# yeyupiaoling/PPASR

Hardware: NVIDIA B200
Metric: utterances_per_sec (higher is better)
Workload: dtype bf16

## Files before the change

### include/ppasr_b200.h

```cpp
#ifndef PPASR_B200_H_
#define PPASR_B200_H_

#include <stdint.h>

#ifdef __cplusplus
extern "C" {
#endif

typedef struct ppasr_b200_ctx ppasr_b200_ctx;

typedef struct ppasr_b200_config {
  int32_t model_type;
  int32_t feat_dim;
  int32_t d_model;
  int32_t n_heads;
  int32_t ffn_dim;
  int32_t n_layers;
  int32_t conv_kernel;
  int32_t causal;
  int32_t conv_norm;
  int32_t vocab_size;
  int32_t max_len;
  int32_t reduce_idx;
  int32_t recover_idx;
// ... 53 lines not shown
int64_t ppasr_b200_beam_workspace_bytes(int32_t B, int32_t T);
int ppasr_b200_beam_reset(void* states, int32_t B, int32_t max_frames, int32_t beam, void* stream);
int ppasr_b200_beam_advance(const float* probs, int32_t B, int32_t T, int32_t V, const int32_t* frame_lens,
                            int32_t beam, float cutoff_prob, int32_t cutoff_top_n, int32_t blank_id, void* states,
                            int32_t max_frames, void* workspace, void* stream);
int ppasr_b200_beam_advance_lm(const float* probs, int32_t B, int32_t T, int32_t V, const int32_t* frame_lens, int32_t beam,
                               float cutoff_prob, int32_t cutoff_top_n, int32_t blank_id, void* states, int32_t max_frames,
                               void* workspace, const uint64_t* lm_keys, const uint32_t* lm_keys_hi, const float* lm_vals,
                               const int32_t* lm_in_vocab, int64_t lm_capacity, int32_t lm_order, float alpha, float beta,
                               void* stream);
int ppasr_b200_beam_result(const void* states, int32_t B, int32_t max_frames, int32_t beam, int32_t* out_ids,
                           int32_t lmax, int32_t* out_lens, float* out_scores, void* stream);
int ppasr_b200_beam_result_nbest(const void* states, int32_t B, int32_t max_frames, int32_t beam, int32_t nbest,
                                 int32_t* out_ids, int32_t lmax, int32_t* out_lens, float* out_scores, void* stream);
int ppasr_b200_op_ctc_prune(const float* probs, int32_t rows, int32_t V, float cutoff_prob, int32_t cutoff_top_n,
                            void* workspace, void* stream);

int ppasr_b200_op_linear(const void* a_bf16, int64_t lda, const void* w_bf16, int64_t w_rows, const float* bias,
                         void* out, int64_t ldo, int32_t M, int32_t N, int32_t K, int32_t epilogue, int32_t act,
                         float alpha, int32_t residual, const int32_t* lens, int32_t T, int32_t block_n, void* stream);
int ppasr_b200_op_layernorm(float* x, void* y_bf16, const float* g1, const float* b1, const float* g2,
                            const float* b2, const int32_t* lens, int32_t T, int32_t M, int32_t D, float eps,
                            void* stream);
int ppasr_b200_op_dwconv(const void* g_bf16, const float* w, const float* bias, const float* pad_left,
                         const float* gamma, const float* beta, int32_t use_layer_norm, void* out_bf16, int32_t B,
                         int32_t Tin, int32_t Tout, int32_t C, int32_t K, int32_t lpad, float eps, void* stream);
int ppasr_b200_op_softmax(const float* logits, int32_t ldl, float* probs, int32_t M, int32_t V, void* stream);
int ppasr_b200_op_fused_ffn(const void* y_bf16, const void* w1_bf16, const void* w2s_bf16, float* x, void* y_out,
                            const float* b1, const float* b2s, const float* g1, const float* bn1, const float* g2,
                            const float* bn2, int32_t M, int32_t FF, float eps, void* stream);
int ppasr_b200_op_attention(const void* q2, const void* kk, const void* vt, int32_t T2p, const void* pos,
                            int32_t pos_rows, int32_t pos_ld, int32_t pos_row0, int32_t pos_col0, void* out,
                            int32_t B, int32_t H, int32_t T1, int32_t T2, const int32_t* klens, void* stream);
int ppasr_b200_op_grouped_attention(const void* q2g, const void* kk, int32_t k_pitch, const void* vt, int32_t vt_pitch,
                                    const void* pos, void* out, int32_t B, int32_t H, int32_t T, int32_t Tgk,
                                    const int32_t* klens, void* stream);

int ppasr_b200_fbank_frames(int32_t n_samples);
int ppasr_b200_fbank(const float* audio, int32_t B, int64_t stride, int32_t N, const int32_t* n_samples, int32_t n_mels,
                     int32_t sample_rate, int32_t db_normalize, float target_db, float* gain_ws, float* out, int32_t Tmax,
                     void* stream);

int ppasr_b200_set_option(ppasr_b200_ctx* ctx, const char* name, int32_t value);

int ppasr_b200_graph_begin(ppasr_b200_ctx* ctx, void* stream);
int ppasr_b200_graph_end(ppasr_b200_ctx* ctx, void* stream);
int ppasr_b200_graph_launch(ppasr_b200_ctx* ctx, void* stream);
int32_t ppasr_b200_graph_kernels(const ppasr_b200_ctx* ctx);

int ppasr_b200_profile_enable(ppasr_b200_ctx* ctx, int32_t enable);
int ppasr_b200_profile_num_classes(void);
const char* ppasr_b200_profile_class_name(int32_t cls);
int ppasr_b200_profile_read(ppasr_b200_ctx* ctx, int32_t* counts, float* total_ms);

int ppasr_b200_debug_copy_x(ppasr_b200_ctx* ctx, float* dst_device, void* stream);
int ppasr_b200_debug_copy_phase(ppasr_b200_ctx* ctx, void* dst_device, int32_t* dims, void* stream);

#ifdef __cplusplus
}
#endif
#endif
```

### ppasr_b200/_lib.py

```python
import ctypes
import os

_HERE = os.path.dirname(os.path.abspath(__file__))
LIB_PATH = os.path.join(_HERE, "lib", "libppasr_b200.so")

c_void_p = ctypes.c_void_p
c_int = ctypes.c_int
c_int64 = ctypes.c_int64
c_float = ctypes.c_float
c_char_p = ctypes.c_char_p

_lib = None


class PPASRB200Error(Exception):
    """Raised when a C-ABI call returns a non-zero status (message from ppasr_b200_last_error)."""


def load():
    global _lib
    if _lib is not None:
        return _lib
    if not os.path.exists(LIB_PATH):
        raise PPASRB200Error(
# ... 26 lines not shown
    "ppasr_b200_destroy": (c_int, [P]),
    "ppasr_b200_load_tensor": (c_int, [P, c_char_p, P, I, P]),
    "ppasr_b200_finalize": (c_int, [P]),
    "ppasr_b200_encode": (c_int, [P, P, I, P, I, I, P]),
    "ppasr_b200_out_frames": (c_int, [P, I]),
    "ppasr_b200_ctc_probs": (c_int, [P, P, I, P]),
    "ppasr_b200_ctc_logits": (c_int, [P, P, I, P]),
    "ppasr_b200_ctc_greedy": (c_int, [P, P, P, P, P, P, I, I, I, P]),
    "ppasr_b200_stream_reset": (c_int, [P, I]),
    "ppasr_b200_encode_chunk": (c_int, [P, P, I, I, I, I, P]),
    "ppasr_b200_stream_info": (c_int, [P, P, P]),
    "ppasr_b200_sessions_init": (c_int, [P, I]),
    "ppasr_b200_sessions_reset": (c_int, [P, I]),
    "ppasr_b200_sessions_step": (c_int, [P, P, I, P, I, I, I, P]),
    "ppasr_b200_fbank_frames": (c_int, [I]),
    "ppasr_b200_fbank": (c_int, [P, I, c_int64, I, P, I, I, I, c_float, P, P, I, P]),
    "ppasr_b200_ds2_states": (c_int, [P, P, P, I, P]),
    "ppasr_b200_stream_export": (c_int, [P, P, P, I, P]),
    "ppasr_b200_beam_state_bytes": (c_int64, [I, I, I]),
    "ppasr_b200_beam_workspace_bytes": (c_int64, [I, I]),
    "ppasr_b200_beam_reset": (c_int, [P, I, I, I, P]),
    "ppasr_b200_beam_advance": (c_int, [P, I, I, I, P, I, c_float, I, I, P, I, P, P]),
    "ppasr_b200_beam_advance_lm": (c_int, [P, I, I, I, P, I, c_float, I, I, P, I, P, P, P, P, P, c_int64, I, c_float, c_float, P]),
    "ppasr_b200_beam_result": (c_int, [P, I, I, I, P, I, P, P, P]),
    "ppasr_b200_beam_result_nbest": (c_int, [P, I, I, I, I, P, I, P, P, P]),
    "ppasr_b200_op_ctc_prune": (c_int, [P, I, I, c_float, I, P, P]),
    "ppasr_b200_greedy_decode": (c_int, [P, I, I, I, P, I, P, I, P, P, P, P, P]),
    "ppasr_b200_op_linear": (c_int, [P, c_int64, P, c_int64, P, P, c_int64, I, I, I, I, I, c_float, I, P, I, I, P]),
    "ppasr_b200_op_layernorm": (c_int, [P, P, P, P, P, P, P, I, I, I, c_float, P]),
    "ppasr_b200_op_dwconv": (c_int, [P, P, P, P, P, P, I, P, I, I, I, I, I, I, c_float, P]),
    "ppasr_b200_op_softmax": (c_int, [P, I, P, I, I, P]),
    "ppasr_b200_op_fused_ffn": (c_int, [P, P, P, P, P, P, P, P, P, P, P, I, I, c_float, P]),
    "ppasr_b200_op_attention": (c_int, [P, P, P, I, P, I, I, I, I, P, I, I, I, I, P, P]),
    "ppasr_b200_op_grouped_attention": (c_int, [P, P, I, P, I, P, P, I, I, I, I, P, P]),
    "ppasr_b200_debug_copy_x": (c_int, [P, P, P]),
    "ppasr_b200_debug_copy_phase": (c_int, [P, P, P, P]),
    "ppasr_b200_set_option": (c_int, [P, c_char_p, I]),
    "ppasr_b200_graph_begin": (c_int, [P, P]),
    "ppasr_b200_graph_end": (c_int, [P, P]),
    "ppasr_b200_graph_launch": (c_int, [P, P]),
    "ppasr_b200_graph_kernels": (c_int, [P]),
    "ppasr_b200_profile_enable": (c_int, [P, I]),
    "ppasr_b200_profile_num_classes": (c_int, []),
    "ppasr_b200_profile_class_name": (c_char_p, [I]),
    "ppasr_b200_profile_read": (c_int, [P, P, P]),
}


def _declare(lib):
    for name, (res, args) in PROTOTYPES.items():
        fn = getattr(lib, name)
        fn.restype = res
        fn.argtypes = args


def ptr(t):
    if t is None:
        return None
    return c_void_p(t.data_ptr())


def stream_ptr(stream=None):
    import torch
    s = stream if stream is not None else torch.cuda.current_stream()
    return c_void_p(s.cuda_stream)
```

### ppasr_b200/csrc/attention.cu

```cuda
#include "kernels.h"
#include "launch.h"
#include "ptx.cuh"

namespace ppasr {

void count_launch();

constexpr int ATT_BM = 128;
constexpr int ATT_BN = 128;
constexpr int ATT_THREADS = 288;
constexpr int ATT_TILE_BYTES = 128 * 64 * 2;
constexpr int ATT_SMEM_Q = 0;
constexpr int ATT_SMEM_KP = 2 * ATT_TILE_BYTES;
constexpr int ATT_SMEM_V = 4 * ATT_TILE_BYTES;
constexpr int ATT_SMEM_BAR = 5 * ATT_TILE_BYTES;
constexpr int ATT_SMEM_XCH = ATT_SMEM_BAR + 128;
constexpr int ATT_SMEM_TOTAL = ATT_SMEM_XCH + 1024 + 1024;
constexpr int ATT_TMEM_COLS = 256;

__global__ void __launch_bounds__(ATT_THREADS, 2)
rel_attention_kernel(const __grid_constant__ CUtensorMap tm_q, const __grid_constant__ CUtensorMap tm_k,
                     const __grid_constant__ CUtensorMap tm_p, const __grid_constant__ CUtensorMap tm_vt,
                     const AttnParams p) {
  extern __shared__ uint8_t smem_raw[];
// ... 175 lines not shown
      const float inv = l_run > 0.f ? 1.0f / l_run : 0.f;
      uint32_t pk[16];
#pragma unroll
      for (int i = 0; i < 16; ++i) pk[i] = pack_bf16x2(o[2 * i] * inv, o[2 * i + 1] * inv);
      uint4* dst = reinterpret_cast<uint4*>(p.out + ((size_t)b * p.T1 + t) * p.D + h * 64 + ch * 32);
#pragma unroll
      for (int i = 0; i < 4; ++i) dst[i] = make_uint4(pk[4 * i], pk[4 * i + 1], pk[4 * i + 2], pk[4 * i + 3]);
    }
  }

  tc_fence_before();
  __syncthreads();
  if (warp_idx == 8) {
    tc_fence_after();
    tmem_dealloc<ATT_TMEM_COLS>(tmem_base);
  }
}

cudaError_t launch_rel_attention(const CUtensorMap& tm_q, const CUtensorMap& tm_k, const CUtensorMap& tm_p,
                                 const CUtensorMap& tm_vt, const AttnParams& p, cudaStream_t st) {
  static bool configured = false;
  if (!configured) {
    cudaError_t e = cudaFuncSetAttribute(rel_attention_kernel, cudaFuncAttributeMaxDynamicSharedMemorySize,
                                         ATT_SMEM_TOTAL);
    if (e != cudaSuccess) return e;
    configured = true;
  }
  dim3 grid((p.T1 + ATT_BM - 1) / ATT_BM, p.H, p.B);
  cudaError_t le = launch_pdl(rel_attention_kernel, grid, dim3(ATT_THREADS), (size_t)ATT_SMEM_TOTAL, st, tm_q, tm_k, tm_p, tm_vt, p);
  count_launch();
  return le != cudaSuccess ? le : cudaGetLastError();
}

}
```

### ppasr_b200/csrc/kernels.h

```cpp
#pragma once
#include <cuda.h>
#include <cuda_bf16.h>
#include <cuda_runtime.h>
#include <stdint.h>

namespace ppasr {

cudaError_t launch_layernorm(float* x, __nv_bfloat16* y, const float* g1, const float* b1, const float* g2,
                             const float* b2, const int* lens, int T, int M, int D, float eps, cudaStream_t st);

cudaError_t launch_conv1_subsample(const float* feats, const float* mean, const float* istd, const float* w,
                                   const float* bias, __nv_bfloat16* out, int B, int T, int F, int C, int T1, int F1,
                                   int Th, int FH, cudaStream_t st);

cudaError_t launch_conv1_tc(const CUtensorMap& tmap_phase, const float* feats, const float* mean, const float* istd,
                            const float* w, const float* bias, int B, int T, int F, int T1, int F1, int Th, int FH,
                            int num_sms, cudaStream_t st);

cudaError_t launch_conv_front_tc(const CUtensorMap& tmap_w2, const float* feats, const float* mean, const float* istd,
                                 const float* w1, const float* b1, const float* b2, __nv_bfloat16* out, int B, int T, int F,
                                 int T1, int F1, int Th, int FH, int Tout, int Fout, int num_sms, cudaStream_t st);

cudaError_t launch_dwconv_norm_swish(const __nv_bfloat16* g, const float* w, const float* bias, const float* pad_left,
                                     const float* gamma, const float* beta, int use_layer_norm, __nv_bfloat16* out,
// ... 69 lines not shown
  float alpha, beta;
};
size_t beam_state_stride(int node_cap);
cudaError_t launch_ctc_prune(const float* probs, int V, int rows, float cutoff_prob, int top_n, int* cnt, int* cid,
                             float* clp, cudaStream_t st);
cudaError_t launch_beam_reset(void* states, int B, int node_cap, cudaStream_t st);
cudaError_t launch_beam_advance(const int* cnt, const int* cid, const float* clp, int B, int T, const int* frame_lens,
                                int beam, int topn, int blank, int max_frames, void* states, int node_cap, cudaStream_t st,
                                const float* probs = nullptr, int V = 0, const BeamLm* lm = nullptr);
cudaError_t launch_beam_result(const void* states, int B, int node_cap, int nbest, int* out_ids, int lmax, int* out_lens,
                               float* out_scores, cudaStream_t st);
constexpr int BEAM_MAX_TOPN = 64;
constexpr int BEAM_MAX_BEAM = 512;

struct AttnParams {
  int B, H;
  int T1;
  int T2;
  int q_rows_per_bh;
  int k_rows_per_bh;
  int k_row0;
  int pos_row0;
  int pos_col0;
  int D;
  const int* klens;
  const int* slots;
  const int* k_row0s;
  const int* pos_row0s;
  __nv_bfloat16* out;
};
cudaError_t launch_rel_attention(const CUtensorMap& tm_q, const CUtensorMap& tm_k, const CUtensorMap& tm_p,
                                 const CUtensorMap& tm_vt, const AttnParams& p, cudaStream_t st);


struct GroupedAttnParams {
  int B, H;
  int T;
  int Tg;
  const int* klens;
  __nv_bfloat16* out;
  int Tgk = 0;
  int k_pitch = 0;
};
cudaError_t launch_grouped_attention(const CUtensorMap& tm_q, const CUtensorMap& tm_k, const CUtensorMap& tm_p,
                                     const CUtensorMap& tm_vt, const GroupedAttnParams& p, cudaStream_t st);
cudaError_t launch_grouped_pos(const __nv_bfloat16* tab, int ldtab, int col0, int T, int Tpad, __nv_bfloat16* out,
                               cudaStream_t st);
cudaError_t launch_dwconv_stride(const __nv_bfloat16* g, const float* w, const float* bias, const float* pad_left,
                                 const float* ng, const float* nb, int layer_norm, __nv_bfloat16* z, int B, int T, int Tout,
                                 int C, int K, int lpad, int stride, float eps, const int* zero_lens, cudaStream_t st);
cudaError_t launch_avgpool2(const float* x, float* out, int B, int T, int Tout, int C, cudaStream_t st);

}
```

### ppasr_b200/csrc/runtime.cu

```cuda
#include <cmath>
#include <cstdlib>
#include <cstring>
#include <map>
#include <string>
#include <vector>

#include "common.h"
#include "gemm.cuh"
#include "kernels.h"
#include "ppasr_b200.h"
#include "tmap.h"

namespace ppasr {

GemmShape make_shape(int M, int N, int K, int block_n);

struct HostTensor {
  std::vector<float> data;
  std::vector<int64_t> shape;
  int64_t numel() const {
    int64_t n = 1;
    for (auto s : shape) n *= s;
    return n;
  }
// ... 6 lines not shown
  cudaError_t reserve(size_t bytes) {
    if (bytes <= cap) return cudaSuccess;
    if (base) cudaFree(base);
    base = nullptr;
    cap = 0;
    cudaError_t e = cudaMalloc(&base, bytes);
    if (e == cudaSuccess) cap = bytes;
    return e;
  }
  void rewind() { used = 0, overflow = false; }
  template <class T>
  T* take(size_t count) {
    const size_t off = (used + 255) & ~size_t(255);
    if (overflow || off + count * sizeof(T) > cap) {
      overflow = true;
      return nullptr;
    }
    used = off + count * sizeof(T);
    return reinterpret_cast<T*>(base + off);
  }
  void release() {
    if (base) cudaFree(base);
    base = nullptr;
    cap = used = 0;
  }
};

struct BlockW {
  const __nv_bfloat16 *wqkv, *wo, *pw1, *pw2;
  const float *bqkv, *bo, *pos_u, *pos_v, *pw1_b, *pw2_b, *dw_w, *dw_b, *cn_g, *cn_b, *glu_pad;
};
struct BlockMaps {
  CUtensorMap wqkv, wo, pw1, pw2;
};

struct LayerW : BlockW {
  const float *ln_ffm_g, *ln_ffm_b, *ln_mha_g, *ln_mha_b, *ln_conv_g, *ln_conv_b, *ln_ff_g, *ln_ff_b, *ln_fin_g,
      *ln_fin_b;
  const __nv_bfloat16 *ffm_w1, *ff_w1, *ffm_w2s, *ff_w2s;
  const float *ffm_b1, *ff_b1, *ffm_b2s, *ff_b2s;
};

struct Plan {
  int B = 0, T = 0, T1 = 0, Tp = 0, Th = 0, M = 0, Mr = 0, Tkp = 0;
  float* feats = nullptr;
  int* vlen = nullptr;
  __nv_bfloat16 *phase = nullptr, *c2 = nullptr, *y = nullptr, *q2 = nullptr, *kk = nullptr, *vt = nullptr,
                *att = nullptr, *g = nullptr, *z = nullptr;
  int Mc = 0, Tc = 0;
  int* vc = nullptr;
  int Tg = 0, Tgp = 0;
  __nv_bfloat16 *q2g = nullptr, *kkg = nullptr, *vtg = nullptr, *pg = nullptr;
  CUtensorMap tm_qg, tm_kg, tm_vtg, tm_pg[4];
  float *x2 = nullptr;
  int* vlen2 = nullptr;
  float *x = nullptr, *logits = nullptr, *pmax = nullptr, *psum = nullptr, *maxp = nullptr, *score = nullptr,
        *probs = nullptr;
  int *parg = nullptr, *idx = nullptr, *ids = nullptr, *out_len = nullptr;
  int Tcat = 0, Mcat = 0;
  __nv_bfloat16 *ycat = nullptr, *gcat = nullptr;
  CUtensorMap tm_phase, tm_c2, tm_y, tm_att, tm_g, tm_z, tm_q, tm_k, tm_vt, tm_ycat;
};

}

using namespace ppasr;
// ... 275 lines not shown
  return PPASR_OK;
}

int pack_attention(ppasr_b200_ctx* c, const std::string& p, int l, bool grouped, bool pos_bias, BlockW& w, BlockMaps& m,
                   std::vector<float>& wpos_all, std::vector<float>& bpos_all) {
  const int D = c->cfg.d_model;
  PPASR_REQUIRE(c->host[p + "self_attn.pos_bias_u"].numel() == (int64_t)c->cfg.n_heads * (grouped ? 192 : 64) &&
                    c->host[p + "self_attn.pos_bias_v"].numel() == (int64_t)c->cfg.n_heads * (grouped ? 192 : 64),
                "pos_bias_u / pos_bias_v shape");
  {
    std::vector<float> qkv((size_t)3 * D * D), bq((size_t)3 * D);
    const char* nm[3] = {"linear_q", "linear_k", "linear_v"};
    for (int s = 0; s < 3; ++s) {
      auto t = transpose_in_out(c->host[p + "self_attn." + nm[s] + ".weight"]);
      std::memcpy(qkv.data() + (size_t)s * D * D, t.data(), sizeof(float) * D * D);
      std::memcpy(bq.data() + (size_t)s * D, c->host[p + "self_attn." + nm[s] + ".bias"].data.data(), sizeof(float) * D);
    }
    w.wqkv = upload(c, to_bf16(qkv));
    w.bqkv = upload(c, bq);
  }
  w.wo = upload(c, to_bf16(transpose_in_out(c->host[p + "self_attn.linear_out.weight"])));
  w.bo = vecf(c, p + "self_attn.linear_out.bias");
  w.pos_u = vecf(c, p + "self_attn.pos_bias_u");
  w.pos_v = vecf(c, p + "self_attn.pos_bias_v");
  {
    auto t = transpose_in_out(c->host[p + "self_attn.linear_pos.weight"]);
    std::memcpy(wpos_all.data() + (size_t)l * D * D, t.data(), sizeof(float) * D * D);
    if (pos_bias)
      std::memcpy(bpos_all.data() + (size_t)l * D, c->host[p + "self_attn.linear_pos.bias"].data.data(), sizeof(float) * D);
  }
  if (int rc = check_weights(c)) return rc;
  std::string err;
  if (!make_tmap_2d(&m.wqkv, w.wqkv, D, 3 * D, (uint64_t)D * 2, BN_NARROW, &err) ||
      !make_tmap_2d(&m.wo, w.wo, D, D, (uint64_t)D * 2, BN_WIDE, &err)) {
    set_last_error(err);
    return PPASR_ERR_CUDA;
  }
  return PPASR_OK;
}

int pack_conv_module(ppasr_b200_ctx* c, const std::string& p, int K, BlockW& w, BlockMaps& m) {
  const auto& cfg = c->cfg;
  const int D = cfg.d_model;
  {
    const HostTensor& pw = c->host[p + "conv_module.pointwise_conv1.weight"];
    const HostTensor& pb = c->host[p + "conv_module.pointwise_conv1.bias"];
    PPASR_REQUIRE(pw.numel() == (int64_t)2 * D * D, "pointwise_conv1.weight shape");
    std::vector<float> wi((size_t)2 * D * D), bi((size_t)2 * D);
    for (int ch = 0; ch < D; ++ch) {
      std::memcpy(&wi[(size_t)(2 * ch) * D], &pw.data[(size_t)ch * D], sizeof(float) * D);
      std::memcpy(&wi[(size_t)(2 * ch + 1) * D], &pw.data[(size_t)(ch + D) * D], sizeof(float) * D);
      bi[2 * ch] = pb.data[ch];
      bi[2 * ch + 1] = pb.data[ch + D];
    }
    w.pw1 = upload(c, to_bf16(wi));
    w.pw1_b = upload(c, bi);
  }
  float* pad = c->wslab.take<float>(D);
  {
    const HostTensor& dw = c->host[p + "conv_module.depthwise_conv.weight"];
    PPASR_REQUIRE(dw.numel() == (int64_t)D * K, "depthwise_conv.weight shape");
    w.dw_w = upload(c, dw.data);
    w.dw_b = vecf(c, p + "conv_module.depthwise_conv.bias");
  }
  if (cfg.conv_norm == 0) {
    w.cn_g = vecf(c, p + "conv_module.norm.weight");
// ... 358 lines not shown
  }
  std::string err;
  bool ok = make_tmap_3d(&n.tm_phase, n.phase, D, n.Mr, 4, (uint64_t)D * 2, (uint64_t)n.Mr * D * 2, GEMM_BLOCK_M, &err) &&
            make_tmap_2d(&n.tm_c2, n.c2, c->Kemb, M, (uint64_t)c->Kemb * 2, GEMM_BLOCK_M, &err) &&
            make_tmap_2d(&n.tm_y, n.y, D, M, (uint64_t)D * 2, GEMM_BLOCK_M, &err) &&
            make_tmap_2d(&n.tm_att, n.att, D, M, (uint64_t)D * 2, GEMM_BLOCK_M, &err) &&
            make_tmap_2d(&n.tm_g, n.g, D, M, (uint64_t)D * 2, GEMM_BLOCK_M, &err) &&
            make_tmap_2d(&n.tm_z, n.z, D, M, (uint64_t)D * 2, GEMM_BLOCK_M, &err) &&
            make_tmap_2d(&n.tm_ycat, n.ycat, D, n.Mcat, (uint64_t)D * 2, GEMM_BLOCK_M, &err) &&
            make_tmap_2d(&n.tm_q, n.q2, 128, (uint64_t)B * H * n.Tp, 256, 128, &err) &&
            make_tmap_2d(&n.tm_k, n.kk, 64, (uint64_t)B * H * n.Tp, 128, 128, &err) &&
            make_tmap_2d(&n.tm_vt, n.vt, n.Tp, (uint64_t)B * H * 64, (uint64_t)n.Tkp * 2, 64, &err);
  if (ok && cfg.model_type == 3) {
    ok = make_tmap_2d(&n.tm_qg, n.q2g, 384, (uint64_t)B * H * n.Tg, 384 * 2, 128, &err) &&
         make_tmap_2d(&n.tm_kg, n.kkg, 192, (uint64_t)B * H * n.Tg, 192 * 2, 64, &err) &&
         make_tmap_2d(&n.tm_vtg, n.vtg, n.Tg, (uint64_t)B * H * 192, (uint64_t)n.Tgp * 2, 192, &err);
    for (int i = 0; ok && i < 4; ++i)
      ok = make_tmap_2d(&n.tm_pg[i], n.pg + (size_t)i * n.Tg * 768, 768, n.Tg, 768 * 2, 64, &err);
  }
  if (!ok) {
    set_last_error(err);
    return PPASR_ERR_CUDA;
  }
  n.Mc = n.M, n.Tc = n.Tp, n.vc = n.vlen;
  if (cfg.model_type == 3 && c->eff_stride_idx >= 0) {
    n.Tc = (n.Tp + 1) / 2;
    n.Mc = B * n.Tc;
    n.vc = n.vlen2;
  }
  p = n;
  return PPASR_OK;
}

template <int BN, int ST, class Epi>
cudaError_t gemm(ppasr_b200_ctx* c, const CUtensorMap& a, const CUtensorMap& b, int M, int N, int K, const Epi& epi,
                 cudaStream_t st) {
  GemmShape s = make_shape(M, N, K, BN);
  return launch_gemm<BN, ST, false>(a, b, s, epi, c->sms, st);
}

int run_subsampling_convs(ppasr_b200_ctx* c, cudaStream_t st) {
  Plan& p = c->plan;
  const auto& cfg = c->cfg;
  const int D = cfg.d_model;
  if (c->fused_conv == 2 && D == 256 && cfg.feat_dim <= 96) {
    PROF(PC_CONV_FRONT);
    PPASR_CUDA_CHECK(launch_conv_front_tc(c->tm_conv2_w, p.feats, c->cmvn_mean, c->cmvn_istd, c->conv1_w, c->conv1_b, c->conv2_b,
                                          p.c2, p.B, p.T, cfg.feat_dim, p.T1, c->F1, p.Th, c->FH, p.Tp, c->F2, c->sms, st));
  } else {
    { PROF(PC_CONV1);
    if (c->conv1_tc && D == 256 && cfg.feat_dim <= 256)
      PPASR_CUDA_CHECK(launch_conv1_tc(p.tm_phase, p.feats, c->cmvn_mean, c->cmvn_istd, c->conv1_w, c->conv1_b, p.B, p.T,
                                       cfg.feat_dim, p.T1, c->F1, p.Th, c->FH, c->sms, st));
    else
      PPASR_CUDA_CHECK(launch_conv1_subsample(p.feats, c->cmvn_mean, c->cmvn_istd, c->conv1_w, c->conv1_b, p.phase, p.B,
                                              p.T, cfg.feat_dim, D, p.T1, c->F1, p.Th, c->FH, st)); }
    GemmShape s = make_shape(p.Mr, D, 9 * D, BN_WIDE);
    s.conv_pitch = c->FH;
    s.conv_kc = D / GEMM_BLOCK_K;
    EpiConv2<BN_WIDE> epi{p.c2, c->conv2_b, p.Mr, D, p.Th, c->FH, p.Tp, c->F2};
    PROF(PC_CONV2);
    PPASR_CUDA_CHECK((launch_gemm<BN_WIDE, ST_WIDE, true>(p.tm_phase, c->tm_conv2_w, s, epi, c->sms, st)));
  }
  return PPASR_OK;
}

// ... 22 lines not shown
  for (int l = 0; l < L; ++l) {
    const LayerW& w = c->layers[l];
    const auto& m = c->lmaps[l];
    const int K = c->layer_k[l];
    const bool grouped = (c->eff_group_mask >> l) & 1;
    const bool strided = l == c->eff_stride_idx;
    {
      PROF(PC_FUSED_FFN);
      PPASR_CUDA_CHECK(launch_fused_ffn(p.tm_y, nullptr, m.ffm_w1_128, m.ffm_w2s, Mc, FF, xc, p.y, w.ffm_b1, w.ffm_b2s, w.ln_mha_g,
                                        w.ln_mha_b, nullptr, nullptr, eps, nullptr, nullptr, nullptr, nullptr, Tc, st));
    }
    const size_t lk = (size_t)l * ss.B * H * ss.Tcap * 64;
    const int kend = ss.kend / rate, kstart = ss.kstart / rate, cache_t = kend - kstart;
    if (grouped && !chunk) {
      PPASR_CUDA_CHECK(launch_grouped_pos(c->pos_tab, L * D, l * D, Tc, 3 * p.Tg, p.pg + (size_t)gi * p.Tg * 768, st));
      EpiQKVGrouped<BN_NARROW> e{p.q2g, p.kkg, p.vtg, w.bqkv, w.pos_u, w.pos_v, Mc, Tc, H, p.Tg, p.Tgp};
      { PROF(PC_QKV); PPASR_CUDA_CHECK((gemm<BN_NARROW, ST_NARROW>(c, p.tm_y, m.wqkv, Mc, 3 * D, D, e, st))); }
      GroupedAttnParams gp{B, H, Tc, p.Tg, vl, p.att};
      { PROF(PC_ATTENTION); PPASR_CUDA_CHECK(launch_grouped_attention(p.tm_qg, p.tm_kg, p.tm_pg[gi], p.tm_vtg, gp, st)); }
      ++gi;
    } else if (grouped) {
      const int T2 = cache_t + Tc, G2 = (T2 + 2) / 3;
      PPASR_CUDA_CHECK(launch_grouped_pos(c->pos_tab, L * D * rate, l * D, T2, 3 * G2, ss.pgc + (size_t)gi * ss.Gcap * 768, st));
      EpiQKVGrouped<BN_NARROW> e{p.q2g, ss.kk + lk, ss.vt + lk, w.bqkv, w.pos_u, w.pos_v, Mc, Tc, H, (Tc + 2) / 3, ss.Gcap};
      e.kofs = kend, e.Tgk = ss.Gcap;
      { PROF(PC_QKV); PPASR_CUDA_CHECK((gemm<BN_NARROW, ST_NARROW>(c, p.tm_y, m.wqkv, Mc, 3 * D, D, e, st))); }
      GroupedAttnParams gp{B, H, Tc, (Tc + 2) / 3, nullptr, p.att};
      gp.Tgk = G2, gp.k_pitch = ss.Gcap;
      { PROF(PC_ATTENTION); PPASR_CUDA_CHECK(launch_grouped_attention(ss.tm_qgc, ss.tm_k[l], ss.tm_pgc[gi], ss.tm_vt[l], gp, st)); }
      ++gi;
    } else {
      AttnParams ap{};
      ap.B = B, ap.H = H, ap.T1 = Tc, ap.D = D, ap.pos_col0 = l * D, ap.out = p.att, ap.q_rows_per_bh = Tc;
      if (!chunk) {
        EpiQKV<BN_NARROW> e{p.q2, p.kk, p.vt, w.bqkv, w.pos_u, w.pos_v, Mc, Tc, H, Tc, p.Tkp, 0};
        { PROF(PC_QKV); PPASR_CUDA_CHECK((gemm<BN_NARROW, ST_NARROW>(c, p.tm_y, m.wqkv, Mc, 3 * D, D, e, st))); }
        ap.T2 = Tc, ap.k_rows_per_bh = Tc, ap.k_row0 = 0, ap.pos_row0 = 0, ap.klens = vl;
        { PROF(PC_ATTENTION); PPASR_CUDA_CHECK(launch_rel_attention(p.tm_q, p.tm_k, *tmpos, p.tm_vt, ap, st)); }
      } else {
        EpiQKV<BN_NARROW> e{p.q2, ss.kk + lk, ss.vt + lk, w.bqkv, w.pos_u, w.pos_v, Mc, Tc, H, ss.Tcap, ss.Tcap, kend};
        if (ss.ragged) e.slots = ss.d_step, e.kofs_b = ss.d_step + B;
        { PROF(PC_QKV); PPASR_CUDA_CHECK((gemm<BN_NARROW, ST_NARROW>(c, p.tm_y, m.wqkv, Mc, 3 * D, D, e, st))); }
        ap.T2 = cache_t + Tc, ap.k_rows_per_bh = ss.Tcap, ap.k_row0 = kstart;
        ap.pos_row0 = (ss.offset - (ss.kend - ss.kstart)) / rate, ap.klens = nullptr;
        if (ss.ragged) {
          ap.T2 = ss.step_T2;
          ap.slots = ss.d_step, ap.k_row0s = ss.d_step + 2 * B, ap.pos_row0s = ss.d_step + 3 * B, ap.klens = ss.d_step + 4 * B;
        }
        { PROF(PC_ATTENTION); PPASR_CUDA_CHECK(launch_rel_attention(p.tm_q, ss.tm_k[l], *tmpos, ss.tm_vt[l], ap, st)); }
      }
    }
    const __nv_bfloat16* gin = p.g;
    int Tin = Tc;
    if (!chunk) {
      PROF(PC_FUSED_ATTN_OUT);
      PPASR_CUDA_CHECK(launch_fused_attn_out(p.tm_att, m.wo, m.pw1, Mc, xc, p.g, w.bo, w.ln_conv_g, w.ln_conv_b, w.pw1_b, vl, Tc,
                                             eps, st));
    } else {
      {
        EpiResidLN<BN_WIDE> e{xc, w.bo, D, Mc, D, 1.0f, 1, nullptr, Tc, 0, 1, w.ln_conv_g, w.ln_conv_b, nullptr, nullptr, p.y, eps};
        PROF(PC_OUTPROJ);
        PPASR_CUDA_CHECK((gemm<BN_WIDE, ST_WIDE>(c, p.tm_att, m.wo, Mc, D, D, e, st)));
      }
      const int lorder = K - 1, Mcat = B * (lorder + Tc);
      PPASR_CUDA_CHECK(launch_conv_cache_concat(ss.cnn + (size_t)l * ss.B * lmax * D, p.y, p.ycat, B, Tc, lorder, D, st,
                                                ss.ragged ? ss.d_step : nullptr));
      EpiGLU<BN_WIDE> eg{p.gcat, w.pw1_b, D, Mcat, 2 * D};
// ... 579 lines not shown
  PPASR_CUDA_CHECK(launch_dwconv_norm_swish((const __nv_bfloat16*)g_bf16, w, bias, pad_left, gamma, beta, use_layer_norm,
                                            (__nv_bfloat16*)out_bf16, B, Tin, Tout, C, K, lpad, eps, nullptr,
                                            reinterpret_cast<cudaStream_t>(stream)));
  return PPASR_OK;
}

int ppasr_b200_op_softmax(const float* logits, int32_t ldl, float* probs, int32_t M, int32_t V, void* stream) {
  PPASR_REQUIRE(logits && probs, "null pointer");
  PPASR_CUDA_CHECK(launch_softmax_rows(logits, ldl, probs, M, V, reinterpret_cast<cudaStream_t>(stream)));
  return PPASR_OK;
}

int ppasr_b200_op_attention(const void* q2, const void* kk, const void* vt, int32_t T2p, const void* pos,
                            int32_t pos_rows, int32_t pos_ld, int32_t pos_row0, int32_t pos_col0, void* out,
                            int32_t B, int32_t H, int32_t T1, int32_t T2, const int32_t* klens, void* stream) {
  PPASR_REQUIRE(q2 && kk && vt && pos && out, "null pointer");
  PPASR_REQUIRE(T2p % 8 == 0 && T2p >= T2 && pos_ld % 8 == 0, "T2p / pos_ld must be multiples of 8");
  std::string err;
  CUtensorMap tq, tk, tp, tv;
  if (!make_tmap_2d(&tq, q2, 128, (uint64_t)B * H * T1, 256, 128, &err) ||
      !make_tmap_2d(&tk, kk, 64, (uint64_t)B * H * T2, 128, 128, &err) ||
      !make_tmap_2d(&tp, pos, pos_ld, pos_rows, (uint64_t)pos_ld * 2, 128, &err) ||
      !make_tmap_2d(&tv, vt, T2, (uint64_t)B * H * 64, (uint64_t)T2p * 2, 64, &err)) {
    set_last_error(err);
    return PPASR_ERR_CUDA;
  }
  AttnParams ap{};
  ap.B = B, ap.H = H, ap.T1 = T1, ap.T2 = T2, ap.q_rows_per_bh = T1, ap.k_rows_per_bh = T2, ap.k_row0 = 0;
  ap.pos_row0 = pos_row0, ap.pos_col0 = pos_col0, ap.D = H * 64, ap.klens = klens, ap.out = (__nv_bfloat16*)out;
  PPASR_CUDA_CHECK(launch_rel_attention(tq, tk, tp, tv, ap, reinterpret_cast<cudaStream_t>(stream)));
  return PPASR_OK;
}

int ppasr_b200_op_grouped_attention(const void* q2g, const void* kk, int32_t k_pitch, const void* vt, int32_t vt_pitch,
                                    const void* pos, void* out, int32_t B, int32_t H, int32_t T, int32_t Tgk,
                                    const int32_t* klens, void* stream) {
  PPASR_REQUIRE(q2g && kk && vt && pos && out, "null pointer");
  PPASR_REQUIRE(B > 0 && H == 4 && T > 0 && Tgk > 0 && k_pitch >= Tgk && vt_pitch >= Tgk, "bad shape (H must be 4)");
  PPASR_REQUIRE(vt_pitch % 8 == 0, "vt_pitch must be a multiple of 8");
  const int Tg = (T + 2) / 3;
  std::string err;
  CUtensorMap tq, tk, tp, tv;
  if (!make_tmap_2d(&tq, q2g, 384, (uint64_t)B * H * Tg, 384 * 2, 128, &err) ||
      !make_tmap_2d(&tk, kk, 192, (uint64_t)B * H * k_pitch, 192 * 2, 64, &err) ||
      !make_tmap_2d(&tp, pos, 768, Tgk, 768 * 2, 64, &err) ||
      !make_tmap_2d(&tv, vt, Tgk, (uint64_t)B * H * 192, (uint64_t)vt_pitch * 2, 192, &err)) {
    set_last_error(err);
    return PPASR_ERR_CUDA;
  }
  GroupedAttnParams gp{B, H, T, Tg, klens, (__nv_bfloat16*)out};
  gp.Tgk = Tgk, gp.k_pitch = k_pitch;
  PPASR_CUDA_CHECK(launch_grouped_attention(tq, tk, tp, tv, gp, reinterpret_cast<cudaStream_t>(stream)));
  return PPASR_OK;
}

}
```

Before: 27390.

## Fuse QKV projection into relative-position attention kernel for short sequences

Adds a single tcgen05 kernel, one CTA per (head, batch), that computes the per-head QKV projection into tensor memory, applies bias and pos_u/pos_v in registers, writes Q/K/V tiles to shared memory, then runs rel-pos flash attention with online softmax. The full-sequence encoder path uses it when D=256, H=4 and T<=256. This replaces a separate QKV GEMM plus attention launch and removes the global round-trip of q2/kk/vt. In exchange, grid size is only B*H CTAs with heavy shared memory and TMEM use, so occupancy may be low for small batches.

```diff
diff --git a/include/ppasr_b200.h b/include/ppasr_b200.h
--- a/include/ppasr_b200.h
+++ b/include/ppasr_b200.h
@@ -109,6 +109,9 @@
 int ppasr_b200_op_attention(const void* q2, const void* kk, const void* vt, int32_t T2p, const void* pos,
                             int32_t pos_rows, int32_t pos_ld, int32_t pos_row0, int32_t pos_col0, void* out,
                             int32_t B, int32_t H, int32_t T1, int32_t T2, const int32_t* klens, void* stream);
+int ppasr_b200_op_qkv_attention(const void* y, const void* wqkv, const float* bqkv, const float* pos_u, const float* pos_v,
+                                const void* pos, int32_t pos_rows, int32_t pos_ld, int32_t pos_row0, int32_t pos_col0,
+                                const int32_t* klens, int32_t B, int32_t T, void* out, int32_t fused, void* stream);
 int ppasr_b200_op_grouped_attention(const void* q2g, const void* kk, int32_t k_pitch, const void* vt, int32_t vt_pitch,
                                     const void* pos, void* out, int32_t B, int32_t H, int32_t T, int32_t Tgk,
                                     const int32_t* klens, void* stream);
diff --git a/ppasr_b200/_lib.py b/ppasr_b200/_lib.py
--- a/ppasr_b200/_lib.py
+++ b/ppasr_b200/_lib.py
@@ -82,6 +82,7 @@
     "ppasr_b200_op_softmax": (c_int, [P, I, P, I, I, P]),
     "ppasr_b200_op_fused_ffn": (c_int, [P, P, P, P, P, P, P, P, P, P, P, I, I, c_float, P]),
     "ppasr_b200_op_attention": (c_int, [P, P, P, I, P, I, I, I, I, P, I, I, I, I, P, P]),
+    "ppasr_b200_op_qkv_attention": (c_int, [P, P, P, P, P, P, I, I, I, I, P, I, I, P, I, P]),
     "ppasr_b200_op_grouped_attention": (c_int, [P, P, I, P, I, P, P, I, I, I, I, P, P]),
     "ppasr_b200_debug_copy_x": (c_int, [P, P, P]),
     "ppasr_b200_debug_copy_phase": (c_int, [P, P, P, P]),
diff --git a/ppasr_b200/csrc/attention.cu b/ppasr_b200/csrc/attention.cu
--- a/ppasr_b200/csrc/attention.cu
+++ b/ppasr_b200/csrc/attention.cu
@@ -231,4 +231,323 @@
   return le != cudaSuccess ? le : cudaGetLastError();
 }
 
+constexpr int QA_THREADS = 544;
+constexpr int QA_W = 0;
+constexpr int QA_Y = 96 * 1024;
+constexpr int QA_POS = 160 * 1024;
+constexpr int QA_Q = 0;
+constexpr int QA_K = 64 * 1024;
+constexpr int QA_V = 96 * 1024;
+constexpr int QA_P1 = 128 * 1024;
+constexpr int QA_BAR = 192 * 1024;
+constexpr int QA_XCH = QA_BAR + 256;
+constexpr int QA_SMEM_TOTAL = QA_XCH + 2048 + 1024;
+constexpr int QA_TMEM_COLS = 512;
+
+__global__ void __launch_bounds__(QA_THREADS, 1)
+qkv_rel_attention_kernel(const __grid_constant__ CUtensorMap tm_y, const __grid_constant__ CUtensorMap tm_w,
+                         const __grid_constant__ CUtensorMap tm_p, const QkvAttnParams p) {
+  extern __shared__ uint8_t smem_raw[];
+  uint8_t* smem = reinterpret_cast<uint8_t*>((reinterpret_cast<uintptr_t>(smem_raw) + 1023) & ~uintptr_t(1023));
+  uint64_t* bar_w = reinterpret_cast<uint64_t*>(smem + QA_BAR);
+  uint64_t* bar_yf = bar_w + 1;
+  uint64_t* bar_ye = bar_w + 5;
+  uint64_t* bar_pos = bar_w + 9;
+  uint64_t* bar_acc = bar_w + 10;
+  uint64_t* bar_qkv = bar_w + 11;
+  uint64_t* bar_s = bar_w + 12;
+  uint64_t* bar_pr = bar_w + 14;
+  uint64_t* bar_o = bar_w + 16;
+  uint32_t* tmem_ptr_smem = reinterpret_cast<uint32_t*>(bar_w + 18);
+
+  const int warp_idx = threadIdx.x >> 5;
+  const int lane = threadIdx.x & 31;
+  const int h = blockIdx.x;
+  const int b = blockIdx.y;
+  const int T = p.T;
+  const int nt = (T + 127) / 128;
+  const int klen = p.klens ? min(T, __ldg(p.klens + b)) : T;
+
+  if (warp_idx == 16) {
+    if (elect_one()) {
+      tma_prefetch_desc(&tm_y);
+      tma_prefetch_desc(&tm_w);
+      tma_prefetch_desc(&tm_p);
+      mbar_init(bar_w, 1);
+      for (int i = 0; i < 4; ++i) {
+        mbar_init(bar_yf + i, 1);
+        mbar_init(bar_ye + i, 1);
+      }
+      mbar_init(bar_pos, 1);
+      mbar_init(bar_acc, 1);
+      mbar_init(bar_qkv, 512);
+      for (int g = 0; g < 2; ++g) {
+        mbar_init(bar_s + g, 1);
+        mbar_init(bar_pr + g, 256);
+        mbar_init(bar_o + g, 1);
+      }
+      fence_barrier_init();
+      fence_proxy_async_smem();
+    }
+    __syncwarp();
+    tmem_alloc<QA_TMEM_COLS>(tmem_ptr_smem);
+  }
+  tc_fence_before();
+  __syncthreads();
+  tc_fence_after();
+  const uint32_t tmem_base = *tmem_ptr_smem;
+  if (warp_idx == 16 && elect_one()) {
+    mbar_arrive_expect_tx(bar_w, 12 * 8192);
+    for (int kb = 0; kb < 4; ++kb)
+      for (int part = 0; part < 3; ++part)
+        tma_load_2d(smem + QA_W + kb * 24576 + part * 8192, &tm_w, bar_w, kb * 64, part * p.D + h * 64);
+  }
+  pdl_wait();
+  pdl_launch_dependents();
+
+  if (warp_idx == 16) {
+    if (elect_one()) {
+      const int row0 = b * T;
+      mbar_arrive_expect_tx(bar_pos, nt * ATT_TILE_BYTES);
+      for (int j = 0; j < nt; ++j)
+        tma_load_2d(smem + QA_POS + j * ATT_TILE_BYTES, &tm_p, bar_pos, p.pos_col0 + h * 64, p.pos_row0 + j * 128);
+      const int nload = nt * 4;
+      for (int i = 0; i < 4 && i < nload; ++i) {
+        mbar_arrive_expect_tx(bar_yf + i, ATT_TILE_BYTES);
+        tma_load_2d(smem + QA_Y + i * ATT_TILE_BYTES, &tm_y, bar_yf + i, i * 64, row0);
+      }
+      constexpr uint32_t idesc_proj = umma_idesc_bf16(128, 192);
+      mbar_wait(bar_w, 0);
+      for (int i = 0; i < nload; ++i) {
+        const int s = i & 3, kb = i & 3, r = i >> 2;
+        mbar_wait(bar_yf + s, (i >> 2) & 1);
+        tc_fence_after();
+        const uint32_t ya = smem_u32(smem + QA_Y + s * ATT_TILE_BYTES), wa = smem_u32(smem + QA_W + kb * 24576);
+#pragma unroll
+        for (int k = 0; k < 4; ++k)
+          umma_bf16(tmem_base + r * 256, umma_desc_k_sw128(ya + k * 32), umma_desc_k_sw128(wa + k * 32), idesc_proj,
+                    (kb | k) != 0);
+        umma_commit(bar_ye + s);
+        if (i >= 1 && i + 3 < nload) {
+          const int ps = (i - 1) & 3, li = i + 3;
+          mbar_wait(bar_ye + ps, ((i - 1) >> 2) & 1);
+          mbar_arrive_expect_tx(bar_yf + ps, ATT_TILE_BYTES);
+          tma_load_2d(smem + QA_Y + ps * ATT_TILE_BYTES, &tm_y, bar_yf + ps, (li & 3) * 64, row0 + (li >> 2) * 128);
+        }
+      }
+      umma_commit(bar_acc);
+      constexpr uint32_t idesc_qk = umma_idesc_bf16(128, 128);
+      constexpr uint32_t idesc_pv = umma_idesc_bf16(128, 64);
+      mbar_wait(bar_pos, 0);
+      mbar_wait(bar_qkv, 0);
+      tc_fence_after();
+      for (int j = 0; j < nt; ++j) {
+        for (int g = 0; g < nt; ++g) {
+          if (j > 0) mbar_wait(bar_o + g, (j - 1) & 1);
+          tc_fence_after();
+          const uint32_t qa = smem_u32(smem + QA_Q + g * 2 * ATT_TILE_BYTES);
+          const uint32_t ka = smem_u32(smem + QA_K + j * ATT_TILE_BYTES), pa = smem_u32(smem + QA_POS + j * ATT_TILE_BYTES);
+          const uint32_t tmem_s = tmem_base + g * 256;
+#pragma unroll
+          for (int k = 0; k < 4; ++k)
+            umma_bf16(tmem_s, umma_desc_k_sw128(qa + k * 32), umma_desc_k_sw128(ka + k * 32), idesc_qk, k > 0);
+#pragma unroll
+          for (int k = 0; k < 4; ++k)
+            umma_bf16(tmem_s, umma_desc_k_sw128(qa + ATT_TILE_BYTES + k * 32), umma_desc_k_sw128(pa + k * 32), idesc_qk, 1u);
+          umma_commit(bar_s + g);
+        }
+        for (int g = 0; g < nt; ++g) {
+          mbar_wait(bar_pr + g, j & 1);
+          tc_fence_after();
+          const uint32_t pt0 = smem_u32(smem + (g == 0 ? QA_K + j * ATT_TILE_BYTES : QA_P1));
+          const uint32_t pt1 = smem_u32(smem + (g == 0 ? QA_POS + j * ATT_TILE_BYTES : QA_P1 + ATT_TILE_BYTES));
+          const uint32_t va = smem_u32(smem + QA_V + j * ATT_TILE_BYTES);
+          const uint32_t tmem_o = tmem_base + g * 256 + 128;
+#pragma unroll
+          for (int kh = 0; kh < 2; ++kh)
+#pragma unroll
+            for (int k = 0; k < 4; ++k)
+              umma_bf16(tmem_o, umma_desc_k_sw128((kh ? pt1 : pt0) + k * 32),
+                        umma_desc_k_sw128(va + kh * (ATT_TILE_BYTES / 2) + k * 32), idesc_pv, (kh | k) != 0);
+          umma_commit(bar_o + g);
+        }
+      }
+    }
+  } else {
+    const int g = warp_idx >> 3;
+    const int quad = warp_idx & 3;
+    const int ch = (warp_idx >> 2) & 1;
+    const int r = quad * 32 + lane;
+    const uint32_t lane_base = ((uint32_t)(quad * 32)) << 16;
+    if (g < nt) {
+      mbar_wait(bar_acc, 0);
+      tc_fence_after();
+      const int hd = h * 64;
+#pragma unroll 1
+      for (int c = 0; c < 3; ++c) {
+        const int cc = ch * 3 + c;
+        const int which = cc >> 1, d0 = (cc & 1) * 32;
+        uint32_t rr[32];
+        tmem_ld_32x32b_x32(tmem_base + lane_base + g * 256 + cc * 32, rr);
+        tmem_ld_wait();
+        float v[32];
+        const float* bias = p.bqkv + which * p.D + hd + d0;
+#pragma unroll
+        for (int j = 0; j < 32; ++j) v[j] = __uint_as_float(rr[j]) + __ldg(bias + j);
+        if (which == 0) {
+          uint8_t* qrow = smem + QA_Q + g * 2 * ATT_TILE_BYTES + r * 128;
+#pragma unroll
+          for (int q4 = 0; q4 < 4; ++q4) {
+            uint32_t pu[4], pv[4];
+#pragma unroll
+            for (int j = 0; j < 4; ++j) {
+              const int e = q4 * 8 + 2 * j;
+              const float2 u = __ldg(reinterpret_cast<const float2*>(p.pos_u + hd + d0 + e));
+              const float2 w = __ldg(reinterpret_cast<const float2*>(p.pos_v + hd + d0 + e));
+              pu[j] = pack_bf16x2(v[e] + u.x, v[e + 1] + u.y);
+              pv[j] = pack_bf16x2(v[e] + w.x, v[e + 1] + w.y);
+            }
+            const int sw = ((d0 >> 3) + q4) ^ (r & 7);
+            *reinterpret_cast<uint4*>(qrow + (sw << 4)) = make_uint4(pu[0], pu[1], pu[2], pu[3]);
+            *reinterpret_cast<uint4*>(qrow + ATT_TILE_BYTES + (sw << 4)) = make_uint4(pv[0], pv[1], pv[2], pv[3]);
+          }
+        } else if (which == 1) {
+          uint8_t* krow = smem + QA_K + g * ATT_TILE_BYTES + r * 128;
+#pragma unroll
+          for (int q4 = 0; q4 < 4; ++q4) {
+            const int e = q4 * 8;
+            const int sw = ((d0 >> 3) + q4) ^ (r & 7);
+            *reinterpret_cast<uint4*>(krow + (sw << 4)) =
+                make_uint4(pack_bf16x2(v[e], v[e + 1]), pack_bf16x2(v[e + 2], v[e + 3]), pack_bf16x2(v[e + 4], v[e + 5]),
+                           pack_bf16x2(v[e + 6], v[e + 7]));
+          }
+        } else {
+          uint8_t* vtile = smem + QA_V + g * ATT_TILE_BYTES + (r >> 6) * (ATT_TILE_BYTES / 2);
+          const int kc = r & 63;
+#pragma unroll
+          for (int j = 0; j < 32; ++j) {
+            const int d = d0 + j;
+            *reinterpret_cast<__nv_bfloat16*>(vtile + d * 128 + ((((kc >> 3) ^ (d & 7))) << 4) + (kc & 7) * 2) =
+                __float2bfloat16_rn(v[j]);
+          }
+        }
+      }
+    }
+    tc_fence_before();
+    fence_proxy_async_smem();
+    mbar_arrive(bar_qkv);
+
+    if (g < nt) {
+      float* xch = reinterpret_cast<float*>(smem + QA_XCH) + g * 256;
+      const uint32_t tmem_s = tmem_base + g * 256, tmem_o = tmem_s + 128;
+      const float sc = 0.125f * 1.4426950408889634f;
+      float m_run = -INFINITY, l_run = 0.f;
+      float o[32];
+#pragma unroll
+      for (int i = 0; i < 32; ++i) o[i] = 0.f;
+
+      for (int j = 0; j < nt; ++j) {
+        const int k0 = j * ATT_BN + ch * 64;
+        mbar_wait(bar_s + g, j & 1);
+        tc_fence_after();
+        float bm = -INFINITY;
+#pragma unroll 1
+        for (int c = 0; c < 2; ++c) {
+          uint32_t rr[32];
+          tmem_ld_32x32b_x32(tmem_s + lane_base + ch * 64 + c * 32, rr);
+          tmem_ld_wait();
+#pragma unroll
+          for (int i = 0; i < 32; ++i) {
+            const bool valid = (k0 + c * 32 + i) < klen;
+            bm = fmaxf(bm, valid ? __uint_as_float(rr[i]) : -INFINITY);
+          }
+        }
+        xch[ch * 128 + r] = bm;
+        named_bar_sync(1 + g, 256);
+        bm = fmaxf(bm, xch[(ch ^ 1) * 128 + r]);
+        const float m_new = fmaxf(m_run, bm * sc);
+        const float m_use = (m_new == -INFINITY) ? 0.f : m_new;
+        const float alpha = exp2f(m_run - m_use);
+        if (g == 0 && nt == 2) mbar_wait(bar_s + 1, j & 1);
+        float bsum = 0.f;
+        uint8_t* tile = smem + (g == 0 ? (ch == 0 ? QA_K : QA_POS) + j * ATT_TILE_BYTES : QA_P1 + ch * ATT_TILE_BYTES) + r * 128;
+#pragma unroll 1
+        for (int c = 0; c < 2; ++c) {
+          uint32_t rr[32];
+          tmem_ld_32x32b_x32(tmem_s + lane_base + ch * 64 + c * 32, rr);
+          tmem_ld_wait();
+          uint32_t pk[16];
+#pragma unroll
+          for (int i = 0; i < 16; ++i) {
+            const int kk0 = k0 + c * 32 + 2 * i;
+            float p0 = (kk0 < klen) ? exp2f(fmaf(__uint_as_float(rr[2 * i]), sc, -m_use)) : 0.f;
+            float p1 = (kk0 + 1 < klen) ? exp2f(fmaf(__uint_as_float(rr[2 * i + 1]), sc, -m_use)) : 0.f;
+            const __nv_bfloat162 pb = __floats2bfloat162_rn(p0, p1);
+            bsum += __low2float(pb) + __high2float(pb);
+            pk[i] = *reinterpret_cast<const uint32_t*>(&pb);
+          }
+#pragma unroll
+          for (int q4 = 0; q4 < 4; ++q4) {
+            const int chunk = c * 4 + q4;
+            *reinterpret_cast<uint4*>(tile + ((chunk ^ (r & 7)) << 4)) =
+                make_uint4(pk[4 * q4], pk[4 * q4 + 1], pk[4 * q4 + 2], pk[4 * q4 + 3]);
+          }
+        }
+        l_run = l_run * alpha + bsum;
+        m_run = m_new;
+        tc_fence_before();
+        fence_proxy_async_smem();
+        mbar_arrive(bar_pr + g);
+        mbar_wait(bar_o + g, j & 1);
+        tc_fence_after();
+        {
+          uint32_t ro[32];
+          tmem_ld_32x32b_x32(tmem_o + lane_base + ch * 32, ro);
+          tmem_ld_wait();
+#pragma unroll
+          for (int i = 0; i < 32; ++i) o[i] = fmaf(o[i], alpha, __uint_as_float(ro[i]));
+        }
+        tc_fence_before();
+        named_bar_sync(1 + g, 256);
+      }
+      xch[ch * 128 + r] = l_run;
+      named_bar_sync(1 + g, 256);
+      l_run += xch[(ch ^ 1) * 128 + r];
+      const int t = g * ATT_BM + r;
+      if (t < T) {
+        const float inv = l_run > 0.f ? 1.0f / l_run : 0.f;
+        uint32_t pk[16];
+#pragma unroll
+        for (int i = 0; i < 16; ++i) pk[i] = pack_bf16x2(o[2 * i] * inv, o[2 * i + 1] * inv);
+        uint4* dst = reinterpret_cast<uint4*>(p.out + ((size_t)b * T + t) * p.D + h * 64 + ch * 32);
+#pragma unroll
+        for (int i = 0; i < 4; ++i) dst[i] = make_uint4(pk[4 * i], pk[4 * i + 1], pk[4 * i + 2], pk[4 * i + 3]);
+      }
+    }
+  }
+
+  tc_fence_before();
+  __syncthreads();
+  if (warp_idx == 16) {
+    tc_fence_after();
+    tmem_dealloc<QA_TMEM_COLS>(tmem_base);
+  }
 }
+
+cudaError_t launch_qkv_rel_attention(const CUtensorMap& tm_y, const CUtensorMap& tm_w, const CUtensorMap& tm_p,
+                                     const QkvAttnParams& p, cudaStream_t st) {
+  if (p.D != 256 || p.H != 4 || p.T < 1 || p.T > 256 || p.B < 1) return cudaErrorInvalidValue;
+  static bool configured = false;
+  if (!configured) {
+    cudaError_t e = cudaFuncSetAttribute(qkv_rel_attention_kernel, cudaFuncAttributeMaxDynamicSharedMemorySize,
+                                         QA_SMEM_TOTAL);
+    if (e != cudaSuccess) return e;
+    configured = true;
+  }
+  cudaError_t le = launch_pdl(qkv_rel_attention_kernel, dim3(p.H, p.B), dim3(QA_THREADS), (size_t)QA_SMEM_TOTAL, st, tm_y,
+                              tm_w, tm_p, p);
+  count_launch();
+  return le != cudaSuccess ? le : cudaGetLastError();
+}
+
+}
diff --git a/ppasr_b200/csrc/kernels.h b/ppasr_b200/csrc/kernels.h
--- a/ppasr_b200/csrc/kernels.h
+++ b/ppasr_b200/csrc/kernels.h
@@ -125,6 +125,19 @@
 cudaError_t launch_rel_attention(const CUtensorMap& tm_q, const CUtensorMap& tm_k, const CUtensorMap& tm_p,
                                  const CUtensorMap& tm_vt, const AttnParams& p, cudaStream_t st);
 
+struct QkvAttnParams {
+  int B, H, T, D;
+  int pos_row0;
+  int pos_col0;
+  const float* bqkv;
+  const float* pos_u;
+  const float* pos_v;
+  const int* klens;
+  __nv_bfloat16* out;
+};
+cudaError_t launch_qkv_rel_attention(const CUtensorMap& tm_y, const CUtensorMap& tm_w, const CUtensorMap& tm_p,
+                                     const QkvAttnParams& p, cudaStream_t st);
+
 
 struct GroupedAttnParams {
   int B, H;
diff --git a/ppasr_b200/csrc/runtime.cu b/ppasr_b200/csrc/runtime.cu
--- a/ppasr_b200/csrc/runtime.cu
+++ b/ppasr_b200/csrc/runtime.cu
@@ -62,6 +62,7 @@
 };
 struct BlockMaps {
   CUtensorMap wqkv, wo, pw1, pw2;
+  CUtensorMap wqkv_h;
 };
 
 struct LayerW : BlockW {
@@ -403,6 +404,7 @@
   if (int rc = check_weights(c)) return rc;
   std::string err;
   if (!make_tmap_2d(&m.wqkv, w.wqkv, D, 3 * D, (uint64_t)D * 2, BN_NARROW, &err) ||
+      !make_tmap_2d(&m.wqkv_h, w.wqkv, D, 3 * D, (uint64_t)D * 2, 64, &err) ||
       !make_tmap_2d(&m.wo, w.wo, D, D, (uint64_t)D * 2, BN_WIDE, &err)) {
     set_last_error(err);
     return PPASR_ERR_CUDA;
@@ -827,6 +829,8 @@
   return PPASR_OK;
 }
 
+bool fused_qkv_attention(int D, int H, int T) { return D == 256 && H == 4 && T >= 1 && T <= 256; }
+
 template <int BN, int ST, class Epi>
 cudaError_t gemm(ppasr_b200_ctx* c, const CUtensorMap& a, const CUtensorMap& b, int M, int N, int K, const Epi& epi,
                  cudaStream_t st) {
@@ -915,7 +919,10 @@
     } else {
       AttnParams ap{};
       ap.B = B, ap.H = H, ap.T1 = Tc, ap.D = D, ap.pos_col0 = l * D, ap.out = p.att, ap.q_rows_per_bh = Tc;
-      if (!chunk) {
+      if (!chunk && fused_qkv_attention(D, H, Tc)) {
+        QkvAttnParams qp{B, H, Tc, D, 0, l * D, w.bqkv, w.pos_u, w.pos_v, vl, p.att};
+        { PROF(PC_ATTENTION); PPASR_CUDA_CHECK(launch_qkv_rel_attention(p.tm_y, m.wqkv_h, *tmpos, qp, st)); }
+      } else if (!chunk) {
         EpiQKV<BN_NARROW> e{p.q2, p.kk, p.vt, w.bqkv, w.pos_u, w.pos_v, Mc, Tc, H, Tc, p.Tkp, 0};
         { PROF(PC_QKV); PPASR_CUDA_CHECK((gemm<BN_NARROW, ST_NARROW>(c, p.tm_y, m.wqkv, Mc, 3 * D, D, e, st))); }
         ap.T2 = Tc, ap.k_rows_per_bh = Tc, ap.k_row0 = 0, ap.pos_row0 = 0, ap.klens = vl;
@@ -1561,6 +1568,61 @@
   return PPASR_OK;
 }
 
+int ppasr_b200_op_qkv_attention(const void* y, const void* wqkv, const float* bqkv, const float* pos_u, const float* pos_v,
+                                const void* pos, int32_t pos_rows, int32_t pos_ld, int32_t pos_row0, int32_t pos_col0,
+                                const int32_t* klens, int32_t B, int32_t T, void* out, int32_t fused, void* stream) {
+  PPASR_REQUIRE(y && wqkv && bqkv && pos_u && pos_v && pos && out, "null pointer");
+  PPASR_REQUIRE(B > 0 && T > 0 && pos_ld % 8 == 0, "bad shape (pos_ld must be a multiple of 8)");
+  const int D = 256, H = 4, M = B * T;
+  cudaStream_t st = reinterpret_cast<cudaStream_t>(stream);
+  std::string err;
+  CUtensorMap ty, tp;
+  if (!make_tmap_2d(&ty, y, D, M, (uint64_t)D * 2, GEMM_BLOCK_M, &err) ||
+      !make_tmap_2d(&tp, pos, pos_ld, pos_rows, (uint64_t)pos_ld * 2, 128, &err)) {
+    set_last_error(err);
+    return PPASR_ERR_CUDA;
+  }
+  if (fused) {
+    CUtensorMap tw;
+    if (!make_tmap_2d(&tw, wqkv, D, 3 * D, (uint64_t)D * 2, 64, &err)) {
+      set_last_error(err);
+      return PPASR_ERR_CUDA;
+    }
+    QkvAttnParams qp{B, H, T, D, pos_row0, pos_col0, bqkv, pos_u, pos_v, klens, (__nv_bfloat16*)out};
+    PPASR_CUDA_CHECK(launch_qkv_rel_attention(ty, tw, tp, qp, st));
+    return PPASR_OK;
+  }
+  const int Tkp = (T + 63) / 64 * 64;
+  __nv_bfloat16 *q2 = nullptr, *kk = nullptr, *vt = nullptr;
+  const size_t nq = (size_t)B * H * T * 128, nk = (size_t)B * H * T * 64, nv = (size_t)B * H * 64 * Tkp;
+  PPASR_CUDA_CHECK(cudaMallocAsync(&q2, (nq + nk + nv) * 2, st));
+  kk = q2 + nq, vt = kk + nk;
+  int rc = PPASR_OK;
+  CUtensorMap tw, tq, tk, tv;
+  if (!make_tmap_2d(&tw, wqkv, D, 3 * D, (uint64_t)D * 2, BN_NARROW, &err) ||
+      !make_tmap_2d(&tq, q2, 128, (uint64_t)B * H * T, 256, 128, &err) ||
+      !make_tmap_2d(&tk, kk, 64, (uint64_t)B * H * T, 128, 128, &err) ||
+      !make_tmap_2d(&tv, vt, T, (uint64_t)B * H * 64, (uint64_t)Tkp * 2, 64, &err)) {
+    set_last_error(err);
+    rc = PPASR_ERR_CUDA;
+  } else {
+    cudaError_t e = cudaMemsetAsync(vt, 0, nv * 2, st);
+    EpiQKV<BN_NARROW> epi{q2, kk, vt, bqkv, pos_u, pos_v, M, T, H, T, Tkp, 0};
+    if (e == cudaSuccess)
+      e = launch_gemm<BN_NARROW, ST_NARROW, false>(ty, tw, make_shape(M, 3 * D, D, BN_NARROW), epi, device_sm_count(), st);
+    AttnParams ap{};
+    ap.B = B, ap.H = H, ap.T1 = T, ap.T2 = T, ap.q_rows_per_bh = T, ap.k_rows_per_bh = T, ap.k_row0 = 0;
+    ap.pos_row0 = pos_row0, ap.pos_col0 = pos_col0, ap.D = D, ap.klens = klens, ap.out = (__nv_bfloat16*)out;
+    if (e == cudaSuccess) e = launch_rel_attention(tq, tk, tp, tv, ap, st);
+    if (e != cudaSuccess) {
+      set_last_error(std::string("CUDA error: ") + cudaGetErrorString(e));
+      rc = PPASR_ERR_CUDA;
+    }
+  }
+  cudaFreeAsync(q2, st);
+  return rc;
+}
+
 int ppasr_b200_op_grouped_attention(const void* q2g, const void* kk, int32_t k_pitch, const void* vt, int32_t vt_pitch,
                                     const void* pos, void* out, int32_t B, int32_t H, int32_t T, int32_t Tgk,
                                     const int32_t* klens, void* stream) {
```

Measured after the change: 29980 (median of 6 runs). +9.4%, better.
